# chenc10/distributed_TensorFlow_models

Measured on AMD Instinct MI355X. Metric: images/sec (whole node) ResNet-50 224×224 bf16 at 1/2/4/8 MI355X, higher is better.
Workload: dtype bf16; 1 GPU; model=resnet_v1_50, global_batch=256, per_gpu_batch=256, image_size=224, parallelism=dp1, device=cuda, grad_allreduce_dtype=fp32, deterministic=True, optimizer=momentum-sgd+wd

## Files before the change

csrc/kernels/conv_igemm.hip:

```cpp
#include "common.h"
#include <cstdio>

namespace dtm {


struct ConvNTArgs {
  const bf16_t* x;
  const bf16_t* w;
  bf16_t* y;
  float* stats;
  const float* bias;
  const float* in_scale;
  const float* in_shift;
  uint32_t x_bytes, w_bytes;
  int N, Hin, Win, C, K, R, S, P, Q;
  int stride, pad_h, pad_w;
  int Hv, Wv;
  int M;
  int Kg;
  int relu;
  FastDiv fd_PQ, fd_Q;
  const bf16_t* add_src;
  int add_stride;
  int add_H, add_W;
// ... 1139 lines not shown
          *(uint2*)(smem + mloc * OROW + kloc * 2) = make_uint2(pack2bf(v[0], v[1]), pack2bf(v[2], v[3]));
        }
    }
  conv_nt_epi_tail<PT, CT, false, false, false, 512, true, false, SPL>(a, smem, p0, c0, by, nullptr, nullptr);
}

template <int CT>
__device__ __forceinline__ void worker_row(float* red, const float* lo, const float* hi, float* row, int c0, int K) {
  constexpr int CPR = CT / 8, RPT = 256 / CPR;
  const int tid = threadIdx.x;
  __syncthreads();
#pragma unroll
  for (int e = 0; e < 8; ++e) { red[tid * 16 + e] = lo[e]; red[tid * 16 + 8 + e] = hi[e]; }
  __syncthreads();
  for (int h = RPT / 2; h >= 1; h >>= 1) {
    if (tid < h * CPR) {
#pragma unroll
      for (int e = 0; e < 16; ++e) red[tid * 16 + e] += red[(tid + h * CPR) * 16 + e];
    }
    __syncthreads();
  }
  const int kc = c0 + tid * 8;
  if (tid < CPR && kc < K) {
#pragma unroll
    for (int e = 0; e < 8; ++e) { row[kc + e] = red[tid * 16 + e]; row[K + kc + e] = red[tid * 16 + 8 + e]; }
  }
}

__device__ __forceinline__ void glds16(const void* gptr, const void* lds) {
  const uint32_t l = __builtin_amdgcn_readfirstlane((uint32_t)(uintptr_t)(const __attribute__((address_space(3))) void*)lds);
  asm volatile("s_mov_b32 m0, %1\n\ts_nop 0\n\tglobal_load_lds_dwordx4 %0, off" ::"v"(gptr), "s"(l) : "memory", "m0");
}

template <int PT, int CT, int NKT, bool PRO, bool STEM = false, int NBUF = 2, bool SIDE = true>
__global__ __launch_bounds__(256) void conv1x1_stream_kernel(ConvNTArgs a, int ntiles) {
  constexpr int WP = PT / 2, WC = CT / 2;
  constexpr int TP = WP / 16, TC = WC / 16;
  constexpr int AI = PT / 32, WI = CT / 32;
  constexpr int ABUF = NKT * PT * 128;
  constexpr int WBUF = NKT * CT * 128;
  constexpr int OROW = CT * 2 + 16;
  constexpr int STG = PT * OROW > 16384 ? PT * OROW : 16384;
  constexpr int NIT = PT * (CT / 8) / 256;
  constexpr int MAXC = 512;
  constexpr int OFF_A = WBUF, OFF_S = WBUF + NBUF * ABUF, OFF_P = OFF_S + STG;
  constexpr int NDMA = NKT * AI;
  static_assert(NBUF == 2 || NBUF == 3, "ring depth");
  static_assert(2 * NIT + NDMA <= 63, "vmcnt range");
  __shared__ __attribute__((aligned(16))) char smem[OFF_P + (PRO ? MAXC * 8 : 0)];
  typedef __attribute__((address_space(1))) const void gvoid;
  typedef __attribute__((address_space(3))) void lvoid;
  static_assert(NIT >= 1 && NIT <= 15, "vmcnt lower bound");

  const int tid = threadIdx.x, lane = tid & 63, wave = tid >> 6;
  const int nb = gridDim.x * gridDim.y;
  const int bid = xcd_remap(blockIdx.y * gridDim.x + blockIdx.x, nb);
  const int bx = bid % gridDim.x, by0 = bid / gridDim.x;
  const int c0 = bx * CT;
  const int lr = lane >> 3;
  const int ch = (lane & 7) ^ lr;
  const char* xg = (const char*)a.x;
  const char* wg = (const char*)a.w;
  const char* zg = (const char*)a.zero;
  float* s_scale = (float*)(smem + OFF_P);
  float* s_shift = s_scale + MAXC;
  if constexpr (PRO) {
    for (int c = tid; c < a.C; c += 256) { s_scale[c] = a.in_scale[c]; s_shift[c] = a.in_shift[c]; }
  }
#pragma unroll
  for (int kt = 0; kt < NKT; ++kt) {
#pragma unroll
    for (int j = 0; j < WI; ++j) {
      const int row = c0 + 8 * (wave + 4 * j) + lr;
      const int k = kt * 64 + ch * 8;
      const bool v = (row < a.K) & (k < a.Kg);
      const char* src = wg + (size_t)(uint32_t)((row * a.Kg + k) * 2);
      __builtin_amdgcn_global_load_lds((gvoid*)(v ? src : zg), (lvoid*)(smem + kt * CT * 128 + (wave + 4 * j) * 1024),
                                       16, 0, 0);
    }
  }
  const char* srcs[NKT * AI];
  auto issue = [&](int t, int buf) {
    char* base = smem + OFF_A + buf * ABUF;
    uint32_t pix[AI];
    if constexpr (STEM) {
#pragma unroll
      for (int j = 0; j < AI; ++j) {
        const int m = t * PT + 8 * (wave + 4 * j) + lr;
        const uint32_t mm = m < a.M ? (uint32_t)m : 0u;
        const uint32_t n = fdiv(mm, a.fd_PQ), rem = mm - n * (a.P * a.Q);
        const uint32_t p = fdiv(rem, a.fd_Q), q = rem - p * a.Q;
        pix[j] = ((n * a.Hin + p * a.stride) * a.Win + q * a.stride) * 8u;
      }
    }
#pragma unroll
    for (int kt = 0; kt < NKT; ++kt) {
      const int k = kt * 64 + ch * 8;
#pragma unroll
      for (int j = 0; j < AI; ++j) {
        const int m = t * PT + 8 * (wave + 4 * j) + lr;
        const bool v = (m < a.M) & (k < a.Kg);
        const char* src = STEM ? xg + (size_t)(pix[j] + (uint32_t)((k >> 5) * a.Win * 8 + (k & 31) * 2))
                               : xg + (size_t)(uint32_t)(m * a.pix_bytes + k * 2);
        srcs[kt * AI + j] = v ? src : zg;
        glds16(srcs[kt * AI + j], base + kt * PT * 128 + (wave + 4 * j) * 1024);
      }
    }
  };
  auto transform = [&](int t, int buf) {
    char* base = smem + OFF_A + buf * ABUF;
#pragma unroll
    for (int kt = 0; kt < NKT; ++kt) {
      const int k = kt * 64 + ch * 8;
      if (k < a.Kg) {
        const float4 s0 = *(const float4*)(s_scale + k), s1 = *(const float4*)(s_scale + k + 4);
        const float4 h0 = *(const float4*)(s_shift + k), h1 = *(const float4*)(s_shift + k + 4);
        const float sc[8] = {s0.x, s0.y, s0.z, s0.w, s1.x, s1.y, s1.z, s1.w};
        const float sh[8] = {h0.x, h0.y, h0.z, h0.w, h1.x, h1.y, h1.z, h1.w};
#pragma unroll
        for (int j = 0; j < AI; ++j) {
          const int m = t * PT + 8 * (wave + 4 * j) + lr;
          if (m < a.M) {
            uint4* pp = (uint4*)(base + kt * PT * 128 + (wave + 4 * j) * 1024 + lane * 16);
            const uint4 q = *pp;
            uint32_t u[4] = {q.x, q.y, q.z, q.w};
#pragma unroll
            for (int e = 0; e < 4; ++e) {
              const float lo = fmaxf(fmaf(lo_bf(u[e]), sc[2 * e], sh[2 * e]), 0.f);
              const float hi = fmaxf(fmaf(hi_bf(u[e]), sc[2 * e + 1], sh[2 * e + 1]), 0.f);
              u[e] = pack2bf(lo, hi);
            }
            *pp = make_uint4(u[0], u[1], u[2], u[3]);
          }
        }
      }
    }
  };

  const int wp = wave % 2, wc = wave / 2;
  const int fr = lane & 15, fk = lane >> 4;
  float ssum[8], ssq[8], aacc[24];
#pragma unroll
  for (int e = 0; e < 8; ++e) { ssum[e] = 0.f; ssq[e] = 0.f; }
#pragma unroll
  for (int e = 0; e < 24; ++e) aacc[e] = 0.f;
  int t = by0;
  const int gy = gridDim.y;
  if (t < ntiles) issue(t, 0);
  if (NBUF == 3 && t + gy < ntiles) issue(t + gy, 1);
  asm volatile("s_waitcnt vmcnt(0)" ::: "memory");
  __syncthreads();
  int buf = 0;
  for (int it = 0; t < ntiles; ++it, t += gy) {
    if constexpr (NBUF == 2) {
      if (it > 0) asm volatile("s_waitcnt vmcnt(%0)" ::"n"(NIT) : "memory");
    } else if (it >= 2) {
      if (t + gy < ntiles) asm volatile("s_waitcnt vmcnt(%0)" ::"n"(2 * NIT + NDMA) : "memory");
      else asm volatile("s_waitcnt vmcnt(%0)" ::"n"(2 * NIT) : "memory");
    }
    if constexpr (PRO) transform(t, buf);
    asm volatile("s_waitcnt lgkmcnt(0)" ::: "memory");
    __builtin_amdgcn_s_barrier();
    if constexpr (NBUF == 2) {
      if (t + gy < ntiles) issue(t + gy, buf ^ 1);
    } else {
      if (t + 2 * gy < ntiles) issue(t + 2 * gy, buf == 0 ? 2 : buf - 1);
    }
    f32x4 acc[TC][TP];
#pragma unroll
    for (int i = 0; i < TC; ++i)
#pragma unroll
      for (int j = 0; j < TP; ++j) acc[i][j] = (f32x4){0.f, 0.f, 0.f, 0.f};
    const char* abase = smem + OFF_A + buf * ABUF;
#pragma unroll
    for (int kt = 0; kt < NKT; ++kt) {
#pragma unroll
      for (int ks = 0; ks < 2; ++ks) {
        short8 bf[TP], af[TC];
        const int chn = ks * 4 + fk;
#pragma unroll
        for (int j = 0; j < TP; ++j) {
          const int row = wp * WP + j * 16 + fr;
          bf[j] = *(const short8*)(abase + kt * PT * 128 + row * 128 + ((chn ^ (row & 7)) << 4));
        }
#pragma unroll
        for (int i = 0; i < TC; ++i) {
          const int row = wc * WC + i * 16 + fr;
          af[i] = *(const short8*)(smem + kt * CT * 128 + row * 128 + ((chn ^ (row & 7)) << 4));
        }
#pragma unroll
        for (int i = 0; i < TC; ++i)
#pragma unroll
          for (int j = 0; j < TP; ++j)
            acc[i][j] = __builtin_amdgcn_mfma_f32_16x16x32_bf16(af[i], bf[j], acc[i][j], 0, 0, 0);
      }
    }
    conv_nt_epilogue<PT, CT, WP, WC, 1, true, true, true, true, 256, SIDE>(a, acc, smem + OFF_S, t * PT, c0, t, ssum,
                                                                           ssq, nullptr, nullptr, aacc);
#pragma unroll
    for (int i = 0; i < NKT * AI; ++i) asm volatile("" ::"v"(srcs[i]));
    buf = buf + 1 == NBUF ? 0 : buf + 1;
  }
  asm volatile("s_waitcnt vmcnt(0)" ::: "memory");
  if (a.stats) worker_row<CT>((float*)(smem + OFF_S), ssum, ssq, a.stats + (size_t)by0 * (2 * a.K), c0, a.K);
  if (SIDE && a.act_x && a.act_sums) {
    const int rw = a.act_r ? 4 : 2;
    float* row = a.act_sums + (size_t)by0 * (rw * a.K);
    worker_row<CT>((float*)(smem + OFF_S), aacc, aacc + 8, row, c0, a.K);
    if (a.act_r) worker_row<CT>((float*)(smem + OFF_S), aacc + 16, aacc + 8, row + 2 * a.K, c0, a.K);
  }
}

template <int CIN>
__device__ __forceinline__ int dsw(int p, int c) {
  return CIN == 64 ? (c ^ ((p >> 1) & 7)) : (c ^ ((p >> 2) & 3));
}

template <int CIN, int CT, bool SIDE>
__global__ __launch_bounds__(256) void conv3x3_direct_kernel(ConvNTArgs a, int ntiles) {
  constexpr int TH = 8, TW = 16, PT = TH * TW, HH = TH + 2, HW = TW + 2;
  constexpr int CPP = CIN / 8;
  constexpr int HCH = HH * HW * CPP;
  constexpr int NDMA = (HCH + 255) / 256;
  constexpr int OROW = CT * 2 + 16;
  constexpr int HDMA = NDMA * 256 * 16;
  constexpr int HBUF = HDMA > PT * OROW ? HDMA : PT * OROW;
  static_assert(3 * HBUF >= 256 * 16 * 4, "worker_row's reduction table fits in the ring");
  constexpr int WBUF = 9 * CT * CIN * 2;
  constexpr int NIT = PT * (CT / 8) / 256;
  constexpr int TC = CT / 16, TP = 2;
  constexpr int SD = SIDE ? 2 * NIT : 0;
  constexpr int SBUF = SIDE ? 2 * NIT * 4096 + 2 * CT * 4 : 0;
  static_assert(2 * NIT + SD + NDMA <= 63, "vmcnt range");
  __shared__ __attribute__((aligned(16))) char smem[WBUF + 3 * HBUF + SBUF];
  char* sside = smem + WBUF + 3 * HBUF;
  float* s_ss = (float*)(sside + 2 * NIT * 4096);

  const int tid = threadIdx.x, lane = tid & 63, wave = tid >> 6;
  const int nb = gridDim.x * gridDim.y;
  const int bid = xcd_remap(blockIdx.y * gridDim.x + blockIdx.x, nb);
  const int bx = bid % gridDim.x, by0 = bid / gridDim.x;
  const int c0 = bx * CT;
// ... 1016 lines not shown
  }
  return (const bf16_t*)z;
}
const void* dtm_zero_chunk() { return zero_chunk(); }

template <int PT, int CT, int NWP, int NS, int UD, bool SPL = false, int NTH = 512>
static void launch_w8(const ConvNTArgs& a, hipStream_t st) {
  dim3 grid((a.K + CT - 1) / CT, (a.M + PT - 1) / PT, a.ngrp > 1 ? a.ngrp : 1);
  hipLaunchKernelGGL((conv_nt_w8_kernel<PT, CT, NWP, NS, UD, SPL, NTH>), grid, dim3(NTH), 0, st, a);
}

template <int UD, bool SPL = false>
static void launch_pp(const ConvNTArgs& a, hipStream_t st) {
  dim3 grid((a.K + 255) / 256, (a.M + 255) / 256, a.ngrp > 1 ? a.ngrp : 1);
  hipLaunchKernelGGL((conv_nt_pp_kernel<UD, SPL>), grid, dim3(512), 0, st, a);
}

template <int PT, int CT, int NS, int UD, int NWP = 2, bool SPL = false>
static void launch_pipe(const ConvNTArgs& a, hipStream_t st) {
  dim3 grid((a.K + CT - 1) / CT, (a.M + PT - 1) / PT, a.ngrp > 1 ? a.ngrp : 1);
  if (SPL) hipLaunchKernelGGL((conv_nt_pipe_kernel<PT, CT, NS, UD, false, NWP, true>), grid, dim3(256), 0, st, a);
  else if (a.in_scale) hipLaunchKernelGGL((conv_nt_pipe_kernel<PT, CT, NS, UD, true, NWP>), grid, dim3(256), 0, st, a);
  else hipLaunchKernelGGL((conv_nt_pipe_kernel<PT, CT, NS, UD, false, NWP>), grid, dim3(256), 0, st, a);
}

static int device_cus() { return dtm_compute_cus(); }

static bf16_t* dump_chunk() {
  static void* z = nullptr;
  if (!z && hipMalloc(&z, 4096) != hipSuccess) return nullptr;
  return (bf16_t*)z;
}

template <int PT, int CT, int NKT, bool PRO, bool STEM = false, int NBUF = 2, bool SIDE = true>
static int stream_workers_k(const ConvNTArgs& a) {
  static int occ = 0;
  if (!occ) {
    if (hipOccupancyMaxActiveBlocksPerMultiprocessor(&occ, conv1x1_stream_kernel<PT, CT, NKT, PRO, STEM, NBUF, SIDE>,
                                                     256, 0) !=
            hipSuccess || occ <= 0)
      occ = 1;
  }
  const int ctiles = (a.K + CT - 1) / CT;
  const int ntiles = (a.M + PT - 1) / PT;
  int workers = (occ * device_cus() + ctiles - 1) / ctiles;
  if (workers > ntiles) workers = ntiles;
  if (workers < 1) workers = 1;
  return workers;
}

template <int PT, int CT, int NKT, bool PRO, bool STEM = false, int NBUF = 2, bool SIDE = true>
static void launch_stream_k(const ConvNTArgs& a, hipStream_t st) {
  const int ctiles = (a.K + CT - 1) / CT;
  const int ntiles = (a.M + PT - 1) / PT;
  hipLaunchKernelGGL((conv1x1_stream_kernel<PT, CT, NKT, PRO, STEM, NBUF, SIDE>),
                     dim3(ctiles, stream_workers_k<PT, CT, NKT, PRO, STEM, NBUF, SIDE>(a)), dim3(256), 0, st, a, ntiles);
}

static bool stem_stream_ok(const ConvNTArgs& a) {
  return a.pix_bytes == 8 && a.C == 32 && a.S == 1 && a.pad_h == 0 && a.pad_w == 0 && a.Kg == a.R * 32 &&
         a.Kg <= 256 && a.K % 64 == 0 && !a.in_scale && !a.bias && !a.relu && a.ostr == 1;
}

template <int CT, int NKT>
static void launch_stream(const ConvNTArgs& a, hipStream_t st) {
  const bool side = a.add_src || a.act_x;
  if (a.in_scale) {
    if (side) launch_stream_k<64, CT, NKT, true, false, 2, true>(a, st);
    else launch_stream_k<64, CT, NKT, true, false, 2, false>(a, st);
  } else if (side) launch_stream_k<64, CT, NKT, false, false, 2, true>(a, st);
  else launch_stream_k<64, CT, NKT, false, false, 2, false>(a, st);
}
template <int CT, int NKT>
static int stream_workers(const ConvNTArgs& a) {
  const bool side = a.add_src || a.act_x;
  if (a.in_scale) return side ? stream_workers_k<64, CT, NKT, true, false, 2, true>(a)
                              : stream_workers_k<64, CT, NKT, true, false, 2, false>(a);
  if (side) return stream_workers_k<64, CT, NKT, false, false, 2, true>(a);
  return stream_workers_k<64, CT, NKT, false, false, 2, false>(a);
}

static int g_stem_stream = 1;
DTM_API void dtm_conv_set_stem_stream(int on) { g_stem_stream = on; }
static int stream_rows(const ConvNTArgs& a, int id) {
  if (id == 33) return g_stem_stream == 2 ? stream_workers_k<64, 64, 4, false, true, 2, false>(a)
                                          : stream_workers_k<64, 64, 4, false, true, 3, false>(a);
  const bool k1 = a.Kg <= 64;
  if (id == 30) {
    return k1 ? stream_workers<128, 1>(a) : stream_workers<128, 2>(a);
  }
  return k1 ? stream_workers<64, 1>(a) : stream_workers<64, 2>(a);
}

static bool stream_ok(const ConvNTArgs& a) {
  return !a.bias && !a.relu && a.R == 1 && a.S == 1 && a.stride == 1 && a.pad_h == 0 && a.pad_w == 0 && a.Hv == a.Hin && a.Wv == a.Win &&
         a.P == a.Hin && a.Q == a.Win && a.Kg % 64 == 0 && a.Kg <= 128 && a.K % 8 == 0 &&
         (!a.in_scale || a.C <= 512) && a.dump != nullptr && a.ostr == 1;
}

template <int PT, int CT, int WP, int WC, int UD, int NBUF = 2, bool SPL = false, int LBW = 0, int EG = 4, int BO = 0>
static void launch_nt(const ConvNTArgs& a, hipStream_t st) {
  dim3 grid((a.K + CT - 1) / CT, (a.M + PT - 1) / PT, a.ngrp > 1 ? a.ngrp : 1);
  hipLaunchKernelGGL((conv_nt_kernel<PT, CT, WP, WC, UD, NBUF, SPL, LBW, EG, BO>), grid, dim3(256), 0, st, a);
}
static int g_act_occ = getenv("DTM_ACT_OCC") ? atoi(getenv("DTM_ACT_OCC")) : 2;
DTM_API void dtm_conv_set_act_occ(int v) { g_act_occ = v; }
static int g_nt_occ = getenv("DTM_NT_OCC") ? atoi(getenv("DTM_NT_OCC")) : 2;
DTM_API void dtm_conv_set_nt_occ(int v) { g_nt_occ = v; }
template <int PT, int CT, int UD>
static void launch_nt_act(const ConvNTArgs& a, hipStream_t st) {
  const bool side = (a.K & 7) == 0 && (a.add_src != nullptr || a.act_x != nullptr);
  const int v = side ? g_act_occ : (a.stats ? 0 : g_nt_occ);
  if (v == 1) launch_nt<PT, CT, 32, 64, UD, 1, false, 0, 2>(a, st);
  else if (v == 2) launch_nt<PT, CT, 32, 64, UD, 1, false, 4, 4>(a, st);
  else if (v == 3) launch_nt<PT, CT, 32, 64, UD, 1, false, 4, 2>(a, st);
  else launch_nt<PT, CT, 32, 64, UD, 1>(a, st);
}

static int g_direct3 = 1;
DTM_API void dtm_conv_set_direct3(int on) { g_direct3 = on; }
static bool direct_ok(const ConvNTArgs& a) {
  return a.R == 3 && a.S == 3 && a.stride == 1 && a.Hv == a.Hin && a.Wv == a.Win && (a.C == 32 || a.C == 64) &&
         a.K % 32 == 0 && !a.in_scale && !a.bias && !a.relu && a.pix_bytes == a.C * 2 && a.ostr == 1 &&
         a.pad_h <= 2 && a.pad_w <= 2 && !a.act_mask && !a.act_r && (!a.add_src || a.add_stride == 1);
}
static void direct_setup(ConvNTArgs& a) {
  a.sp_tw = (a.Q + 15) / 16;
  a.sp_th = (a.P + 7) / 8;
  a.fd_sp_img = make_fastdiv(a.sp_th * a.sp_tw);
// ... 15 lines not shown
}
template <int CIN, int CT, bool SIDE>
static void launch_direct_k(const ConvNTArgs& a, hipStream_t st) {
  hipLaunchKernelGGL((conv3x3_direct_kernel<CIN, CT, SIDE>), dim3(a.K / CT, direct_workers_k<CIN, CT, SIDE>(a)),
                     dim3(256), 0, st, a, a.M / 128);
}
static int g_direct_ct32 = getenv("DTM_DIRECT_CT32") ? atoi(getenv("DTM_DIRECT_CT32")) : 1;
DTM_API void dtm_conv_set_direct_ct32(int on) { g_direct_ct32 = on; }
#define DTM_DIRECT_SEL(FN, ...)                                                                     \
  ((a.add_src || a.act_x)                                                                          \
       ? (a.C == 64 ? FN<64, 32, true>(__VA_ARGS__) : FN<32, 32, true>(__VA_ARGS__))                 \
       : (a.C == 64 ? ((a.K % 64 == 0 && !g_direct_ct32) ? FN<64, 64, false>(__VA_ARGS__)           \
                                                        : FN<64, 32, false>(__VA_ARGS__))           \
                    : ((a.K % 64 == 0 && !g_direct_ct32) ? FN<32, 64, false>(__VA_ARGS__)           \
                                                        : FN<32, 32, false>(__VA_ARGS__))))
static int direct_workers(const ConvNTArgs& a) { return DTM_DIRECT_SEL(direct_workers_k, a); }
static void launch_direct(const ConvNTArgs& a, hipStream_t st) { DTM_DIRECT_SEL(launch_direct_k, a, st); }

struct TileCfg {
  int id, PT, NWP;
};
static int g_tile_env = -2;
static int g_last_nt_tile = -1, g_last_wgrad_tile = -1;
DTM_API void dtm_conv_last_tiles(int* nt, int* wgrad) {
  if (nt) *nt = g_last_nt_tile;
  if (wgrad) *wgrad = g_last_wgrad_tile;
}
static int device_cus();
static int g_policy2 = 1;
DTM_API void dtm_conv_set_policy2(int on) { g_policy2 = on; }
static int g_tile_w8 = 1;
static int g_stream_act = 0;
DTM_API void dtm_conv_set_stream_act(int on) { g_stream_act = on; }
static int g_kwide = 1;
DTM_API void dtm_conv_set_kwide(int on) { g_kwide = on; }
DTM_API void dtm_conv_set_w8(int on) { g_tile_w8 = on; }
static int g_tile_pp = getenv("DTM_PP") ? atoi(getenv("DTM_PP")) : 0;
DTM_API void dtm_conv_set_pp(int on) { g_tile_pp = on; }
static int g_k64_tile = 3;
DTM_API void dtm_conv_set_k64_tile(int id) { g_k64_tile = id; }
static int g_k32_tile = 1;
DTM_API void dtm_conv_set_k32(int on) { g_k32_tile = on; }
static int g_act_tile = -1;
DTM_API void dtm_conv_set_act_tile(int id) { g_act_tile = id; }
static TileCfg pick_tile_impl(const ConvNTArgs& a, bool stats);
static TileCfg pick_tile(const ConvNTArgs& a, bool stats = false) {
  static int log = -1;
  if (log < 0) {
    const char* e = getenv("DTM_TILE_LOG");
    log = e ? atoi(e) : 0;
  }
  const TileCfg t = pick_tile_impl(a, stats);
  if (log)
    fprintf(stderr, "dtm_tile M=%d K=%d C=%d RxS=%dx%d Kg=%d st=%d ostr=%d pro=%d stats=%d add=%d act=%d mask=%d r=%d -> %d\n",
            a.M, a.K, a.C, a.R, a.S, a.Kg, a.stride, a.ostr, a.in_scale != nullptr, (int)stats, a.add_src != nullptr,
            a.act_x != nullptr, a.act_mask != nullptr, a.act_r != nullptr, t.id);
  return t;
}
static TileCfg pick_tile_impl(const ConvNTArgs& a, bool stats) {
  if (g_tile_env == -2) {
    const char* e = getenv("DTM_CONV_TILE");
    g_tile_env = e ? atoi(e) : -1;
  }
  int id = g_tile_env;
  if (id == -1 && g_stem_stream && stem_stream_ok(a)) return {33, 64, 2};
  if (((id == -1 && a.K == 32) || id == 60) && g_direct3 && direct_ok(a)) return {60, 128, 4};
  if (id == -1 && a.K == 64 && a.C == 32 && !a.in_scale && g_direct3 && direct_ok(a)) return {60, 128, 4};
  if (id == -4) id = -1;
  else if (id == -1 && a.Kg == 64 && stream_ok(a) && (g_stream_act || !a.act_x) &&
           (!g_policy2 || a.K % 128 == 0 || a.K <= 64))
    id = a.K >= 128 ? 30 : 31;
  if (id == -1 && a.act_x && g_act_tile >= 0) id = g_act_tile;
  if (id == -1 && !a.in_scale && a.K >= 256 && g_tile_w8 && (!g_policy2 || a.K % 256 == 0)) {
    const long tiles = (long)((a.M + 255) / 256) * ((a.K + 255) / 256);
    if (tiles >= 150 && !(tiles > 600 && a.Kg <= 256 && !stats)) id = 40;
  }
  if (id == -1 && g_policy2 && !a.in_scale && a.K % 8 == 0 && a.R * a.S > 1) {
    if (a.K <= 32 && g_k32_tile) id = 32;
    else if (a.K <= 64) id = 26;
    else if (a.K <= 128) id = 21;
  }
  if (id == -1 && g_kwide && a.K > 64 && a.K % 128 != 0 && (a.K % 128) <= 64 && a.K % 8 == 0)
    id = a.in_scale ? 3 : ((g_policy2 && a.M >= 16384 && (a.M <= 65536 || a.M >= 262144)) ? 24 : 26);
  if (id == -1 && !a.in_scale && a.Kg >= 1024) {
    id = 21;
    if (g_policy2 && (long)((a.M + 127) / 128) * ((a.K + 127) / 128) <= device_cus()) id = 26;
  }
  if (id == -1 && !a.in_scale && a.K <= 64 && a.R * a.S > 1 && a.K % 64 == 0) id = 26;
  if (id < 0) id = a.K <= 64 ? g_k64_tile : ((a.M <= 16384 && a.Kg >= 2048) ? 0 : 4);
  if ((id == 21 || id == 24 || id == 26 || id == 32) && a.in_scale && a.C > 512) id = 0;
  if (id == 21 || id == 26) return {id, 128, 2};
  if (id == 24) return {id, 256, 2};
  if (id == 32) return {id, 256, 4};
  if ((id == 40 || id == 41) && a.in_scale) id = 0;
  if (id == 40 && g_tile_pp && g_tile_env != 40) id = 41;
  if (id == 41 && a.K % 8) id = 40;
  if (id == 40 || id == 41) return {id, 256, 2};
  if (id == 30 || id == 31) {
    if (stream_ok(a)) return {id, 64, 2};
    id = a.K <= 64 ? 3 : 4;
  }
  if (id == 3) return {id, 128, 4};
  if (id == 4) return {id, 64, 2};
  return {0, 128, 2};
}

static void dispatch_split(const ConvNTArgs& a, const TileCfg& t, hipStream_t st) {
  const int id = t.id;
  g_last_nt_tile = (id == 3 || id == 4 || id == 21 || id == 24 || id == 26 || id == 32 || id == 40 || id == 41) ? id : 0;
  if (t.id == 3) launch_nt<128, 64, 32, 64, 1, 1, true>(a, st);
  else if (t.id == 4) launch_nt<64, 128, 32, 64, 1, 1, true>(a, st);
  else if (t.id == 21) launch_pipe<128, 128, 2, 1, 2, true>(a, st);
  else if (t.id == 24) launch_pipe<256, 64, 2, 1, 2, true>(a, st);
  else if (t.id == 26) launch_pipe<128, 64, 2, 1, 2, true>(a, st);
  else if (t.id == 32) launch_pipe<256, 32, 2, 1, 4, true>(a, st);
  else if (t.id == 40) launch_w8<256, 256, 2, 2, 1, true>(a, st);
  else if (t.id == 41) launch_pp<1, true>(a, st);
  else launch_nt<128, 128, 64, 64, 1, 2, true>(a, st);
}

template <int UD>
static void dispatch_ud(const ConvNTArgs& a, const TileCfg& t, hipStream_t st) {
  if (UD == 1 && a.nsplit > 0) dispatch_split(a, t, st);
  else if (t.id == 3) launch_nt_act<128, 64, UD>(a, st);
  else if (t.id == 4) launch_nt_act<64, 128, UD>(a, st);
  else if (t.id == 30 && UD == 1) {
    if (a.Kg <= 64) launch_stream<128, 1>(a, st);
    else launch_stream<128, 2>(a, st);
  } else if (t.id == 60 && UD == 1) {
    launch_direct(a, st);
  } else if (t.id == 33 && UD == 1) {
    if (g_stem_stream == 2) launch_stream_k<64, 64, 4, false, true, 2, false>(a, st);
    else launch_stream_k<64, 64, 4, false, true, 3, false>(a, st);
  } else if (t.id == 31 && UD == 1) {
    if (a.Kg <= 64) launch_stream<64, 1>(a, st);
    else launch_stream<64, 2>(a, st);
  } else if (t.id == 21) launch_pipe<128, 128, 2, UD>(a, st);
  else if (t.id == 24) launch_pipe<256, 64, 2, UD>(a, st);
  else if (t.id == 26) launch_pipe<128, 64, 2, UD>(a, st);
  else if (t.id == 32) launch_pipe<256, 32, 2, UD, 4>(a, st);
  else if (t.id == 40) launch_w8<256, 256, 2, 2, UD>(a, st);
  else if (t.id == 41) launch_pp<UD>(a, st);
  else launch_nt<128, 128, 64, 64, UD>(a, st);
}

DTM_API void dtm_conv_set_tile(int id) { g_tile_env = id; }

static void dispatch_nt(const ConvNTArgs& a, int ud, const TileCfg& t, hipStream_t st) {
  g_last_nt_tile = (ud != 1 && (t.id == 30 || t.id == 31 || t.id == 33 || t.id == 60)) ? 0 : t.id;
  if (ud == 1) dispatch_ud<1>(a, t, st);
  else dispatch_ud<2>(a, t, st);
}

DTM_API int dtm_get_deterministic();

static int g_split_tile = 1;
DTM_API void dtm_conv_set_split_tile(int on) { g_split_tile = on; }

static int g_blockout = -1, g_blockout_nt = 1;
DTM_API void dtm_conv_set_blockout(int mode, int nt) { g_blockout = mode; g_blockout_nt = nt; }
struct BlockOut {
  const void* res;
  const float* ss;
  const float* rss;
  void* y;
  void* mask;
};
constexpr int DTM_DECLINED = 1;
static void launch_blockout(const ConvNTArgs& a, int tile, hipStream_t st) {
  g_last_nt_tile = tile == 3 ? 3 : 4;
  if (tile == 3) {
    if (g_blockout_nt) launch_nt<128, 64, 32, 64, 1, 1, false, 3, 4, 2>(a, st);
    else launch_nt<128, 64, 32, 64, 1, 1, false, 3, 4, 1>(a, st);
  } else {
    if (g_blockout_nt) launch_nt<64, 128, 32, 64, 1, 1, false, 3, 4, 2>(a, st);
    else launch_nt<64, 128, 32, 64, 1, 1, false, 3, 4, 1>(a, st);
  }
}

static int conv_fwd_impl(const void* x, const void* w, void* y, bool stats, const float* bias, const float* in_scale,
                         const float* in_shift, int relu, const ConvDesc* d, hipStream_t stream, float** rows_ws,
                         int* nrows, const ConvNTArgs::Split* split = nullptr, int nsplit = 0,
// ... 2 lines not shown
  if (d->C % 8 || d->K % 4) return -1;
  ConvNTArgs a;
  a.x = (const bf16_t*)x; a.w = (const bf16_t*)w; a.y = (bf16_t*)y;
  a.ngrp = 0;
  a.nsplit = 0;
  a.stats = nullptr; a.bias = bias; a.in_scale = in_scale; a.in_shift = in_shift;
  a.add_src = nullptr; a.act_x = nullptr; a.act_ss = nullptr; a.act_sums = nullptr;
  a.act_mask = nullptr; a.act_r = nullptr;
  a.add_stride = 1; a.add_H = a.add_W = 0;
  a.act_unscaled = 0;
  a.zero = zero_chunk();
  a.dump = dump_chunk();
  a.pix_bytes = d->pix_bytes > 0 ? d->pix_bytes : d->C * 2;
  size_t xb = (size_t)d->N * d->H * d->W * a.pix_bytes, wb = (size_t)d->K * d->R * d->S * d->C * 2;
  if (xb >= (1ull << 31) || wb >= (1ull << 31)) return -2;
  a.x_bytes = (uint32_t)xb; a.w_bytes = (uint32_t)wb;
  a.N = d->N; a.Hin = d->H; a.Win = d->W; a.C = d->C; a.K = d->K; a.R = d->R; a.S = d->S;
  a.P = d->P; a.Q = d->Q; a.stride = d->stride; a.pad_h = d->pad_h; a.pad_w = d->pad_w;
  a.Hv = d->H; a.Wv = d->W;
  a.M = d->N * d->P * d->Q; a.Kg = d->R * d->S * d->C; a.relu = relu;
  a.fd_PQ = make_fastdiv(d->P * d->Q); a.fd_Q = make_fastdiv(d->Q);
  a.ostr = 1; a.oa = a.ob = 0; a.OH = a.P; a.OW = a.Q;
  a.sp_tw = a.sp_th = 0;
  if (nsplit > 0) {
    if (nsplit > 8 || d->K % 8) return -1;
    a.nsplit = nsplit;
    for (int i = 0; i < nsplit; ++i) {
      if (split[i].off % 8 || split[i].K % 8) return -1;
      a.split[i] = split[i];
    }
  }
  int rows = 0;
  TileCfg tc = pick_tile(a, stats);
  if (nsplit > 0 && (tc.id == 30 || tc.id == 31 || tc.id == 33 || tc.id == 60)) tc = {4, 64, 2};
  if (nsplit > 0 && g_split_tile && g_tile_env < 0 && tc.id != 40 && tc.id != 21) tc = {21, 128, 2};
  if (bo) {
    const int ct = tc.id == 3 ? 64 : 128;
    if (g_blockout == 0 || (tc.id != 3 && tc.id != 4) || (g_blockout == 2 && tc.id != 3) ||
        (g_blockout == 3 && tc.id != 4) || a.K > ct || a.R != 1 || a.S != 1 || a.stride != 1 ||
        a.pad_h || a.pad_w || a.P != a.Hin || a.Q != a.Win || a.C % 8 || a.C > 512 || a.pix_bytes != a.C * 2 ||
        bias || relu || in_scale || nsplit > 0 || !stats || !bo->res || !bo->ss || !bo->y)
      return DTM_DECLINED;
    a.bo_res = (const bf16_t*)bo->res; a.bo_ss = bo->ss; a.bo_rss = bo->rss;
    a.bo_y = (bf16_t*)bo->y; a.bo_mask = (uint8_t*)bo->mask;
  }
  if (tc.id == 60) direct_setup(a);
  if (stats) {
    rows = tc.id == 60 ? direct_workers(a)
           : (tc.id == 30 || tc.id == 31 || tc.id == 33) ? stream_rows(a, tc.id)
                                                          : ((a.M + tc.PT - 1) / tc.PT) * ((a.K & 7) == 0 ? 1 : tc.NWP);
    float* ws = dtm_ws_get_stream((size_t)rows * 2 * d->K, stream);
    if (!ws) return -4;
    a.stats = ws;
  }
  if (bo) launch_blockout(a, tc.id, stream);
  else dispatch_nt(a, 1, tc, stream);
  *rows_ws = a.stats;
  *nrows = rows;
  return 0;
}

DTM_API int dtm_conv_fwd(const void* x, const void* w, void* y, float* stats, const float* bias,
                         const float* in_scale, const float* in_shift, int relu,
                         const ConvDesc* d, void* stream) {
  float* ws = nullptr;
  int rows = 0;
  int rc = conv_fwd_impl(x, w, y, stats != nullptr, bias, in_scale, in_shift, relu, d, (hipStream_t)stream, &ws, &rows);
  if (rc) return rc;
  if (stats) dtm_reduce_rows(ws, rows, 2 * d->K, 2 * d->K, stats, (hipStream_t)stream);
  return 0;
}

DTM_API int dtm_conv_fwd_bn_multi(const void* x, const void* w, void* const* ys, const int* ks, int n,
                                  void* const* bn_ptrs, float count, float eps, float decay, int update, int bessel,
                                  const ConvDesc* d, void* stream) {
  if (n < 1 || n > 8) return -1;
  ConvNTArgs::Split sp[8];
  FinGroup fg;
  fg.n = n;
  int off = 0;
  for (int i = 0; i < n; ++i) {
    sp[i].y = (bf16_t*)ys[i];
// ... 102 lines not shown
  const int st = d->stride;
  const bool dec = d->dec && st > 1;
  if (!dec && st > 2) return -3;
  if (dec && (d->R < st || d->S < st)) return -8;
  ConvNTArgs la[16];
  TileCfg lt[16];
  int lrows[16], nl = 0, rows = 0;
  for (int ca = 0; ca < (dec ? st : 1); ++ca)
    for (int cb = 0; cb < (dec ? st : 1); ++cb) {
      ConvNTArgs b = a;
      if (dec) {
        int r0, Tr, offa, s0, Tu, offb;
        dec_dim(d->R, st, d->pad_h, ca, r0, Tr, offa);
        dec_dim(d->S, st, d->pad_w, cb, s0, Tu, offb);
        const int Hc = (d->H - ca + st - 1) / st, Wc = (d->W - cb + st - 1) / st;
        if (Hc <= 0 || Wc <= 0) continue;
        b.w = (const bf16_t*)wt + dec_block(d->R, d->S, d->C, d->K, st, d->pad_h, d->pad_w, ca, cb);
        b.R = Tr; b.S = Tu;
        b.P = Hc; b.Q = Wc;
        b.pad_h = Tr - 1 - offa; b.pad_w = Tu - 1 - offb;
        b.ostr = st; b.oa = ca; b.ob = cb;
      } else {
        b.R = d->R; b.S = d->S;
        b.P = d->H; b.Q = d->W;
        b.pad_h = d->R - 1 - d->pad_h; b.pad_w = d->S - 1 - d->pad_w;
        b.Hv = (d->P - 1) * st + 1; b.Wv = (d->Q - 1) * st + 1;
        b.ostr = 1; b.oa = b.ob = 0;
      }
      b.M = d->N * b.P * b.Q; b.Kg = b.R * b.S * d->K;
      b.fd_PQ = make_fastdiv(b.P * b.Q); b.fd_Q = make_fastdiv(b.Q);
      lt[nl] = pick_tile(b);
      if (lt[nl].id == 60) direct_setup(b);
      lrows[nl] = lt[nl].id == 60 ? direct_workers(b)
                  : (lt[nl].id == 30 || lt[nl].id == 31) ? stream_rows(b, lt[nl].id)
                                                         : (b.M + lt[nl].PT - 1) / lt[nl].PT;
      rows += lrows[nl];
      la[nl++] = b;
    }
  int gi = -1;
  if (dec && nl > 1 && nl <= 4 && g_dec_group) {
    gi = 0;
    for (int i = 1; i < nl; ++i) {
      if (la[i].M != la[0].M || la[i].P != la[0].P || la[i].Q != la[0].Q) gi = -2;
      if (gi >= 0 && la[i].Kg > la[gi].Kg) gi = i;
    }
    int id = gi >= 0 ? lt[gi].id : -1;
    if (gi >= 0 && g_dec_tile && (id == 21 || id == 26) && g_tile_env < 0 && g_act_tile < 0) {
      if (la[gi].K % 256 == 0 && g_tile_w8) lt[gi] = {g_tile_pp ? 41 : 40, 256, 2};
      else if (la[gi].K <= 128) lt[gi] = {26, 128, 2};
      id = lt[gi].id;
    }
    if (!(id == 0 || id == 3 || id == 4 || id == 21 || id == 24 || id == 26 || id == 32 || id == 40 || id == 41)) gi = -1;
    if (gi >= 0) {
      rows = 0;
      for (int i = 0; i < nl; ++i) {
        lt[i] = lt[gi];
        lrows[i] = (la[i].M + lt[gi].PT - 1) / lt[gi].PT;
        rows += lrows[i];
      }
    }
  }
  float* ws = nullptr;
  if (act_x) {
    ws = dtm_ws_get_stream((size_t)rows * rw * d->C, (hipStream_t)stream);
    if (!ws) return -4;
  }
  for (int i = 0, r = 0; i < nl; r += lrows[i], ++i)
// ... 257 lines not shown
```

distributed_tensorflow_models_amd/ops/_lib.py:

```python
import ctypes
import os

import torch

_HERE = os.path.dirname(os.path.dirname(os.path.abspath(__file__)))
LIB_PATH = os.environ.get("DTM_KERNELS_SO") or os.path.join(_HERE, "_native", "libdtm_kernels.so")

_lib = None


class ConvDesc(ctypes.Structure):
    _fields_ = [(n, ctypes.c_int) for n in
                ("N", "H", "W", "C", "K", "R", "S", "P", "Q", "stride", "pad_h", "pad_w", "pix_bytes", "dec")]


class PoolArgs(ctypes.Structure):
    _fields_ = [(n, ctypes.c_int) for n in
                ("N", "H", "W", "C", "P", "Q", "KH", "KW", "SH", "SW", "PH", "PW")]


_P = ctypes.c_void_p
_I = ctypes.c_int
_L = ctypes.c_long
_F = ctypes.c_float
# ... 110 lines not shown
    "dtm_bn_finalize_bwd": (None, [_P, _P, _P, _P, _P, _P, _I, _F, _P]),
    "dtm_lrn": (_I, [_P, _P, _P, _L, _I, _I, _F, _F, _F, _I, _P]),
    "dtm_ws_reserve": (_I, [_L]),
    "dtm_ws_last_error": (_I, []),
    "dtm_ws_retired": (_L, []),
    "dtm_ws_reserve_stream": (_I, [_L, _P]),
    "dtm_ws_capacity": (_L, [_P]),
    "dtm_depthwise_fwd": (_I, [_P, _P, _P, _P, _P]),
    "dtm_depthwise_dgrad": (_I, [_P, _P, _P, _P, _P]),
    "dtm_depthwise_wgrad": (_I, [_P, _P, _P, _P, _P]),
    "dtm_set_reduce_policy": (None, [_I, _I, _I]),
    "dtm_bn_apply_ld": (_I, [_P, _P, _P, _P, _L, _I, _I, _I, _P]),
    "dtm_bn_apply_bwd_ld": (_I, [_P, _P, _P, _P, _P, _P, _L, _I, _I, _I, _P]),
    "dtm_set_sc_policy": (None, [_I, _I]),
    "dtm_set_ntld_policy": (None, [_I]),
    "dtm_set_deterministic": (None, [_I]),
    "dtm_get_deterministic": (_I, []),
    "dtm_conv_set_k64_tile": (None, [_I]),
    "dtm_conv_set_w8": (None, [_I]),
    "dtm_conv_set_kwide": (None, [_I]),
    "dtm_set_reduce_few": (None, [_I]),
    "dtm_set_reserved_cus": (None, [_I]),
    "dtm_stats_combine_multi": (_I, [_P, _P, _I, _F, _P, _L, _I, _P]),
    "dtm_conv_fwd_bn_multi": (_I, [_P, _P, _P, _P, _I, _P, _F, _F, _F, _I, _I, ctypes.POINTER(ConvDesc), _P]),
    "dtm_conv_fwd_bn_blockout": (_I, [_P] * 13 + [_F, _F, _F, _I, _I, ctypes.POINTER(ConvDesc), _P]),
    "dtm_conv_set_blockout": (None, [_I, _I]),
    "dtm_conv_set_dec_lpt": (None, [_I]),
    "dtm_conv_set_dec_tile": (None, [_I]),
    "dtm_conv_set_split_tile": (None, [_I]),
    "dtm_get_reserved_cus": (_I, []),
    "dtm_compute_cus_api": (_I, []),
    "dtm_cu_hog": (_I, [_I, _F, _P]),
    "dtm_conv_set_stream_act": (None, [_I]),
    "dtm_conv_set_act_tile": (None, [_I]),
    "dtm_stem_pack": (_I, [_P, _I, _P, _I, _I, _I, _I, _I, _I, _I, _P]),
    "dtm_dropout": (_I, [_P, _P, _L, _I, _F, ctypes.c_ulonglong, _P, _P]),
    "dtm_in_top_k": (_I, [_P, _P, _P, _I, _I, _I, _I, _P]),
    "dtm_stats_tensor_bytes": (_I, []),
    "dtm_stats_chunk_bytes": (_I, []),
    "dtm_stats_partial_bytes": (_I, []),
    "dtm_stats_result_bytes": (_I, []),
    "dtm_stats_chunk_size": (_I, []),
    "dtm_stats_num_buckets": (_I, []),
    "dtm_stats_limits": (None, [_P]),
    "dtm_tensor_stats": (_I, [_P, _P, _I, _I, _P, _P, _P, _P]),
    "dtm_metrics_header_words": (_I, []),
    "dtm_metrics_max_classes": (_I, []),
    "dtm_metrics_max_confusion_classes": (_I, []),
    "dtm_metrics_max_batch": (_I, []),
    "dtm_eval_metrics": (_I, [_P, _I, _P, _I, _I, _I, _I, _I, _P, _P, _P, _P]),
    "dtm_fq_rec_words": (_I, []),
    "dtm_fq_partial_stride": (_I, []),
    "dtm_fq_threads": (_I, []),
    "dtm_fq_grid": (_I, [_L, _I]),
    "dtm_fq_range": (_I, [_P, _I, _L, _P, _P]),
    "dtm_fq_finalize": (_I, [_P, _I, _P, _P, _P, _P, _I, _F, _F, _I, _I, _L, _I, _P]),
    "dtm_fq_apply": (_I, [_P, _P, _I, _L, _P, _P]),
    "dtm_fq_apply_bwd": (_I, [_P, _P, _P, _I, _L, _P, _P]),
    "dtm_fq_advance": (_I, [_P, _P]),
}


def gpu_present():
    try:
        return torch.cuda.is_available()
    except Exception:
# ... 138 lines not shown
```

Measured before the change: 15730 images/sec.

## Add 8-wave persistent stream 1x1 conv kernel for Kg 128/256 with grouped stats rows

Generalizes the streaming 1x1 conv kernel to 512 threads (8 waves) and adds two new tile ids (34, 35) that use it for 1x1 convs with Kg 128 or 256 and K divisible by 256. Each worker walks groups of four 64-row tiles and writes one deterministic BN-stats row per 256 output rows, so stats match the existing 256-row partition. The weight tile stays resident in LDS while activation tiles stream through a double buffer. This aims to cut the weight reloads and tile launch overhead of the generic tiled path. In exchange it adds per-group reductions and barriers, and it uses more LDS per block.

```diff
diff --git a/csrc/kernels/conv_igemm.hip b/csrc/kernels/conv_igemm.hip
--- a/csrc/kernels/conv_igemm.hip
+++ b/csrc/kernels/conv_igemm.hip
@@ -1195,18 +1195,25 @@
   asm volatile("s_mov_b32 m0, %1\n\ts_nop 0\n\tglobal_load_lds_dwordx4 %0, off" ::"v"(gptr), "s"(l) : "memory", "m0");
 }
 
-template <int PT, int CT, int NKT, bool PRO, bool STEM = false, int NBUF = 2, bool SIDE = true>
-__global__ __launch_bounds__(256) void conv1x1_stream_kernel(ConvNTArgs a, int ntiles) {
-  constexpr int WP = PT / 2, WC = CT / 2;
+template <int PT, int CT, int NKT, bool PRO, bool STEM = false, int NBUF = 2, bool SIDE = true, int NT = 256>
+__global__ __launch_bounds__(NT) void conv1x1_stream_kernel(ConvNTArgs a, int ntiles) {
+  constexpr int NW = NT / 64;
+  static_assert(NT == 256 || (NT == 512 && !SIDE && !STEM), "4 waves, or the 8-wave forward form");
+  constexpr int WP = PT / 2, WC = CT / (NW / 2);
   constexpr int TP = WP / 16, TC = WC / 16;
-  constexpr int AI = PT / 32, WI = CT / 32;
+  constexpr int AI = PT / (8 * NW), WI = CT / (8 * NW);
+  static_assert(AI >= 1 && WI >= 1 && PT % (8 * NW) == 0 && CT % (8 * NW) == 0, "whole DMA pieces per wave");
   constexpr int ABUF = NKT * PT * 128;
   constexpr int WBUF = NKT * CT * 128;
   constexpr int OROW = CT * 2 + 16;
   constexpr int STG = PT * OROW > 16384 ? PT * OROW : 16384;
-  constexpr int NIT = PT * (CT / 8) / 256;
+  constexpr int NIT = PT * (CT / 8) / NT;
   constexpr int MAXC = 512;
   constexpr int OFF_A = WBUF, OFF_S = WBUF + NBUF * ABUF, OFF_P = OFF_S + STG;
+  constexpr bool TR = NT == 512;
+  constexpr int NSTAT = (CT / 8) * 16;
+  static_assert(!TR || (NBUF == 2 && PT == 64 && NSTAT <= NT && STG >= NSTAT * 64), "group rows: table in the staging area");
+  static_assert(OFF_P + (PRO ? MAXC * 8 : 0) <= 160 * 1024, "LDS budget");
   constexpr int NDMA = NKT * AI;
   static_assert(NBUF == 2 || NBUF == 3, "ring depth");
   static_assert(2 * NIT + NDMA <= 63, "vmcnt range");
@@ -1228,17 +1235,17 @@
   float* s_scale = (float*)(smem + OFF_P);
   float* s_shift = s_scale + MAXC;
   if constexpr (PRO) {
-    for (int c = tid; c < a.C; c += 256) { s_scale[c] = a.in_scale[c]; s_shift[c] = a.in_shift[c]; }
+    for (int c = tid; c < a.C; c += NT) { s_scale[c] = a.in_scale[c]; s_shift[c] = a.in_shift[c]; }
   }
 #pragma unroll
   for (int kt = 0; kt < NKT; ++kt) {
 #pragma unroll
     for (int j = 0; j < WI; ++j) {
-      const int row = c0 + 8 * (wave + 4 * j) + lr;
+      const int row = c0 + 8 * (wave + NW * j) + lr;
       const int k = kt * 64 + ch * 8;
       const bool v = (row < a.K) & (k < a.Kg);
       const char* src = wg + (size_t)(uint32_t)((row * a.Kg + k) * 2);
-      __builtin_amdgcn_global_load_lds((gvoid*)(v ? src : zg), (lvoid*)(smem + kt * CT * 128 + (wave + 4 * j) * 1024),
+      __builtin_amdgcn_global_load_lds((gvoid*)(v ? src : zg), (lvoid*)(smem + kt * CT * 128 + (wave + NW * j) * 1024),
                                        16, 0, 0);
     }
   }
@@ -1249,7 +1256,7 @@
     if constexpr (STEM) {
 #pragma unroll
       for (int j = 0; j < AI; ++j) {
-        const int m = t * PT + 8 * (wave + 4 * j) + lr;
+        const int m = t * PT + 8 * (wave + NW * j) + lr;
         const uint32_t mm = m < a.M ? (uint32_t)m : 0u;
         const uint32_t n = fdiv(mm, a.fd_PQ), rem = mm - n * (a.P * a.Q);
         const uint32_t p = fdiv(rem, a.fd_Q), q = rem - p * a.Q;
@@ -1261,12 +1268,12 @@
       const int k = kt * 64 + ch * 8;
 #pragma unroll
       for (int j = 0; j < AI; ++j) {
-        const int m = t * PT + 8 * (wave + 4 * j) + lr;
+        const int m = t * PT + 8 * (wave + NW * j) + lr;
         const bool v = (m < a.M) & (k < a.Kg);
         const char* src = STEM ? xg + (size_t)(pix[j] + (uint32_t)((k >> 5) * a.Win * 8 + (k & 31) * 2))
                                : xg + (size_t)(uint32_t)(m * a.pix_bytes + k * 2);
         srcs[kt * AI + j] = v ? src : zg;
-        glds16(srcs[kt * AI + j], base + kt * PT * 128 + (wave + 4 * j) * 1024);
+        glds16(srcs[kt * AI + j], base + kt * PT * 128 + (wave + NW * j) * 1024);
       }
     }
   };
@@ -1282,9 +1289,9 @@
         const float sh[8] = {h0.x, h0.y, h0.z, h0.w, h1.x, h1.y, h1.z, h1.w};
 #pragma unroll
         for (int j = 0; j < AI; ++j) {
-          const int m = t * PT + 8 * (wave + 4 * j) + lr;
+          const int m = t * PT + 8 * (wave + NW * j) + lr;
           if (m < a.M) {
-            uint4* pp = (uint4*)(base + kt * PT * 128 + (wave + 4 * j) * 1024 + lane * 16);
+            uint4* pp = (uint4*)(base + kt * PT * 128 + (wave + NW * j) * 1024 + lane * 16);
             const uint4 q = *pp;
             uint32_t u[4] = {q.x, q.y, q.z, q.w};
 #pragma unroll
@@ -1307,14 +1314,15 @@
   for (int e = 0; e < 8; ++e) { ssum[e] = 0.f; ssq[e] = 0.f; }
 #pragma unroll
   for (int e = 0; e < 24; ++e) aacc[e] = 0.f;
-  int t = by0;
   const int gy = gridDim.y;
+  int t = TR ? 4 * by0 : by0;
+  auto nxt = [&](int u) { return TR ? ((u & 3) == 3 ? u + 4 * gy - 3 : u + 1) : u + gy; };
   if (t < ntiles) issue(t, 0);
   if (NBUF == 3 && t + gy < ntiles) issue(t + gy, 1);
   asm volatile("s_waitcnt vmcnt(0)" ::: "memory");
   __syncthreads();
   int buf = 0;
-  for (int it = 0; t < ntiles; ++it, t += gy) {
+  for (int it = 0; t < ntiles; ++it, t = nxt(t)) {
     if constexpr (NBUF == 2) {
       if (it > 0) asm volatile("s_waitcnt vmcnt(%0)" ::"n"(NIT) : "memory");
     } else if (it >= 2) {
@@ -1325,7 +1333,7 @@
     asm volatile("s_waitcnt lgkmcnt(0)" ::: "memory");
     __builtin_amdgcn_s_barrier();
     if constexpr (NBUF == 2) {
-      if (t + gy < ntiles) issue(t + gy, buf ^ 1);
+      if (nxt(t) < ntiles) issue(nxt(t), buf ^ 1);
     } else {
       if (t + 2 * gy < ntiles) issue(t + 2 * gy, buf == 0 ? 2 : buf - 1);
     }
@@ -1358,19 +1366,68 @@
             acc[i][j] = __builtin_amdgcn_mfma_f32_16x16x32_bf16(af[i], bf[j], acc[i][j], 0, 0, 0);
       }
     }
-    conv_nt_epilogue<PT, CT, WP, WC, 1, true, true, true, true, 256, SIDE>(a, acc, smem + OFF_S, t * PT, c0, t, ssum,
-                                                                           ssq, nullptr, nullptr, aacc);
+    float dsum[8], dsq[8];
+#pragma unroll
+    for (int e = 0; e < 8; ++e) { dsum[e] = 0.f; dsq[e] = 0.f; }
+    constexpr bool OWN = TR && CT != 256;
+    conv_nt_epilogue<PT, CT, WP, WC, 1, true, true, true, true, NT, SIDE>(a, acc, smem + OFF_S, t * PT, c0, t,
+                                                                          OWN ? dsum : ssum, OWN ? dsq : ssq, nullptr,
+                                                                          nullptr, aacc);
+    if constexpr (TR) {
+      if (a.stats) {
+        constexpr int CPR = CT / 8;
+        if constexpr (OWN) {
+          if (tid < NSTAT) {
+            const int c = tid % CPR, g = tid / CPR;
+            const int kc = c0 + c * 8;
+#pragma unroll
+            for (int j = 0; j < 4; ++j) {
+              const int row = g + 16 * j;
+              if (t * PT + row < a.M && kc < a.K) {
+                const uint4 v = *(const uint4*)(smem + OFF_S + row * OROW + c * 16);
+                const float q[8] = {lo_bf(v.x), hi_bf(v.x), lo_bf(v.y), hi_bf(v.y),
+                                    lo_bf(v.z), hi_bf(v.z), lo_bf(v.w), hi_bf(v.w)};
+#pragma unroll
+                for (int e = 0; e < 8; ++e) { ssum[e] += q[e]; ssq[e] = fmaf(q[e], q[e], ssq[e]); }
+              }
+            }
+          }
+        }
+        if ((t & 3) == 3) {
+          epi_barrier<true>();
+          float* red = (float*)(smem + OFF_S);
+          if (tid < NSTAT) {
+#pragma unroll
+            for (int e = 0; e < 8; ++e) { red[tid * 16 + e] = ssum[e]; red[tid * 16 + 8 + e] = ssq[e]; }
+          }
+          epi_barrier<true>();
+          float* prow = a.stats + (size_t)(t >> 2) * (2 * a.K);
+          for (int o = tid; o < CPR * 16; o += NT) {
+            const int c = o >> 4, e = o & 15;
+            float r = 0.f;
+#pragma unroll 4
+            for (int k = 0; k < 16; ++k) r += red[((c + k * CPR) << 4) + e];
+            const int kk = c0 + c * 8 + (e & 7);
+            if (kk < a.K) prow[(e < 8 ? 0 : a.K) + kk] = r;
+          }
+#pragma unroll
+          for (int e = 0; e < 8; ++e) { ssum[e] = 0.f; ssq[e] = 0.f; }
+        }
+      }
+    }
 #pragma unroll
     for (int i = 0; i < NKT * AI; ++i) asm volatile("" ::"v"(srcs[i]));
     buf = buf + 1 == NBUF ? 0 : buf + 1;
   }
   asm volatile("s_waitcnt vmcnt(0)" ::: "memory");
-  if (a.stats) worker_row<CT>((float*)(smem + OFF_S), ssum, ssq, a.stats + (size_t)by0 * (2 * a.K), c0, a.K);
-  if (SIDE && a.act_x && a.act_sums) {
-    const int rw = a.act_r ? 4 : 2;
-    float* row = a.act_sums + (size_t)by0 * (rw * a.K);
-    worker_row<CT>((float*)(smem + OFF_S), aacc, aacc + 8, row, c0, a.K);
-    if (a.act_r) worker_row<CT>((float*)(smem + OFF_S), aacc + 16, aacc + 8, row + 2 * a.K, c0, a.K);
+  if constexpr (!TR) {
+    if (a.stats) worker_row<CT>((float*)(smem + OFF_S), ssum, ssq, a.stats + (size_t)by0 * (2 * a.K), c0, a.K);
+    if (SIDE && a.act_x && a.act_sums) {
+      const int rw = a.act_r ? 4 : 2;
+      float* row = a.act_sums + (size_t)by0 * (rw * a.K);
+      worker_row<CT>((float*)(smem + OFF_S), aacc, aacc + 8, row, c0, a.K);
+      if (a.act_r) worker_row<CT>((float*)(smem + OFF_S), aacc + 16, aacc + 8, row + 2 * a.K, c0, a.K);
+    }
   }
 }
 
@@ -2453,29 +2510,32 @@
   return (bf16_t*)z;
 }
 
-template <int PT, int CT, int NKT, bool PRO, bool STEM = false, int NBUF = 2, bool SIDE = true>
+static int g_stream_workers_cap = 0;
+DTM_API void dtm_conv_set_stream_workers_cap(int n) { g_stream_workers_cap = n; }
+template <int PT, int CT, int NKT, bool PRO, bool STEM = false, int NBUF = 2, bool SIDE = true, int NT = 256>
 static int stream_workers_k(const ConvNTArgs& a) {
   static int occ = 0;
   if (!occ) {
-    if (hipOccupancyMaxActiveBlocksPerMultiprocessor(&occ, conv1x1_stream_kernel<PT, CT, NKT, PRO, STEM, NBUF, SIDE>,
-                                                     256, 0) !=
+    if (hipOccupancyMaxActiveBlocksPerMultiprocessor(&occ, conv1x1_stream_kernel<PT, CT, NKT, PRO, STEM, NBUF, SIDE, NT>,
+                                                     NT, 0) !=
             hipSuccess || occ <= 0)
       occ = 1;
   }
   const int ctiles = (a.K + CT - 1) / CT;
-  const int ntiles = (a.M + PT - 1) / PT;
+  const int ntiles = NT == 512 ? (a.M + 255) / 256 : (a.M + PT - 1) / PT;
   int workers = (occ * device_cus() + ctiles - 1) / ctiles;
+  if (g_stream_workers_cap > 0 && workers > g_stream_workers_cap) workers = g_stream_workers_cap;
   if (workers > ntiles) workers = ntiles;
   if (workers < 1) workers = 1;
   return workers;
 }
 
-template <int PT, int CT, int NKT, bool PRO, bool STEM = false, int NBUF = 2, bool SIDE = true>
+template <int PT, int CT, int NKT, bool PRO, bool STEM = false, int NBUF = 2, bool SIDE = true, int NT = 256>
 static void launch_stream_k(const ConvNTArgs& a, hipStream_t st) {
   const int ctiles = (a.K + CT - 1) / CT;
-  const int ntiles = (a.M + PT - 1) / PT;
-  hipLaunchKernelGGL((conv1x1_stream_kernel<PT, CT, NKT, PRO, STEM, NBUF, SIDE>),
-                     dim3(ctiles, stream_workers_k<PT, CT, NKT, PRO, STEM, NBUF, SIDE>(a)), dim3(256), 0, st, a, ntiles);
+  const int ntiles = NT == 512 ? 4 * ((a.M + 255) / 256) : (a.M + PT - 1) / PT;
+  hipLaunchKernelGGL((conv1x1_stream_kernel<PT, CT, NKT, PRO, STEM, NBUF, SIDE, NT>),
+                     dim3(ctiles, stream_workers_k<PT, CT, NKT, PRO, STEM, NBUF, SIDE, NT>(a)), dim3(NT), 0, st, a, ntiles);
 }
 
 static bool stem_stream_ok(const ConvNTArgs& a) {
@@ -2501,9 +2561,16 @@
   return stream_workers_k<64, CT, NKT, false, false, 2, false>(a);
 }
 
+template <int CT, int NKT>
+static void launch_stream8(const ConvNTArgs& a, hipStream_t st) {
+  if (a.in_scale) launch_stream_k<64, CT, NKT, true, false, 2, false, 512>(a, st);
+  else launch_stream_k<64, CT, NKT, false, false, 2, false, 512>(a, st);
+}
+
 static int g_stem_stream = 1;
 DTM_API void dtm_conv_set_stem_stream(int on) { g_stem_stream = on; }
 static int stream_rows(const ConvNTArgs& a, int id) {
+  if (id == 34 || id == 35) return (a.M + 255) / 256;
   if (id == 33) return g_stem_stream == 2 ? stream_workers_k<64, 64, 4, false, true, 2, false>(a)
                                           : stream_workers_k<64, 64, 4, false, true, 3, false>(a);
   const bool k1 = a.Kg <= 64;
@@ -2513,9 +2580,11 @@
   return k1 ? stream_workers<64, 1>(a) : stream_workers<64, 2>(a);
 }
 
-static bool stream_ok(const ConvNTArgs& a) {
+static bool stream_ok(const ConvNTArgs& a, int id = 30) {
+  const int kmax = id == 35 ? 256 : 128;
+  if ((id == 34 || id == 35) && (a.add_src || a.act_x)) return false;
   return !a.bias && !a.relu && a.R == 1 && a.S == 1 && a.stride == 1 && a.pad_h == 0 && a.pad_w == 0 && a.Hv == a.Hin && a.Wv == a.Win &&
-         a.P == a.Hin && a.Q == a.Win && a.Kg % 64 == 0 && a.Kg <= 128 && a.K % 8 == 0 &&
+         a.P == a.Hin && a.Q == a.Win && a.Kg % 64 == 0 && a.Kg <= kmax && a.K % 8 == 0 &&
          (!a.in_scale || a.C <= 512) && a.dump != nullptr && a.ostr == 1;
 }
 
@@ -2597,6 +2666,8 @@
 static int g_tile_w8 = 1;
 static int g_stream_act = 0;
 DTM_API void dtm_conv_set_stream_act(int on) { g_stream_act = on; }
+static int g_stream8 = 3;
+DTM_API void dtm_conv_set_stream8(int classes) { g_stream8 = classes; }
 static int g_kwide = 1;
 DTM_API void dtm_conv_set_kwide(int on) { g_kwide = on; }
 DTM_API void dtm_conv_set_w8(int on) { g_tile_w8 = on; }
@@ -2635,6 +2706,10 @@
   else if (id == -1 && a.Kg == 64 && stream_ok(a) && (g_stream_act || !a.act_x) &&
            (!g_policy2 || a.K % 128 == 0 || a.K <= 64))
     id = a.K >= 128 ? 30 : 31;
+  else if (id == -1 && stats && !a.in_scale && g_tile_w8 && a.K % 256 == 0 &&
+           (long)((a.M + 255) / 256) * (a.K / 256) >= 150 &&
+           (((g_stream8 & 1) && a.Kg == 128 && stream_ok(a, 34)) || ((g_stream8 & 2) && a.Kg == 256 && stream_ok(a, 35))))
+    id = a.Kg == 128 ? 34 : 35;
   if (id == -1 && a.act_x && g_act_tile >= 0) id = g_act_tile;
   if (id == -1 && !a.in_scale && a.K >= 256 && g_tile_w8 && (!g_policy2 || a.K % 256 == 0)) {
     const long tiles = (long)((a.M + 255) / 256) * ((a.K + 255) / 256);
@@ -2661,8 +2736,8 @@
   if (id == 40 && g_tile_pp && g_tile_env != 40) id = 41;
   if (id == 41 && a.K % 8) id = 40;
   if (id == 40 || id == 41) return {id, 256, 2};
-  if (id == 30 || id == 31) {
-    if (stream_ok(a)) return {id, 64, 2};
+  if (id == 30 || id == 31 || id == 34 || id == 35) {
+    if (stream_ok(a, id)) return {id, 64, 2};
     id = a.K <= 64 ? 3 : 4;
   }
   if (id == 3) return {id, 128, 4};
@@ -2692,6 +2767,10 @@
   else if (t.id == 30 && UD == 1) {
     if (a.Kg <= 64) launch_stream<128, 1>(a, st);
     else launch_stream<128, 2>(a, st);
+  } else if (t.id == 34 && UD == 1) {
+    launch_stream8<256, 2>(a, st);
+  } else if (t.id == 35 && UD == 1) {
+    launch_stream8<128, 4>(a, st);
   } else if (t.id == 60 && UD == 1) {
     launch_direct(a, st);
   } else if (t.id == 33 && UD == 1) {
@@ -2712,7 +2791,7 @@
 DTM_API void dtm_conv_set_tile(int id) { g_tile_env = id; }
 
 static void dispatch_nt(const ConvNTArgs& a, int ud, const TileCfg& t, hipStream_t st) {
-  g_last_nt_tile = (ud != 1 && (t.id == 30 || t.id == 31 || t.id == 33 || t.id == 60)) ? 0 : t.id;
+  g_last_nt_tile = (ud != 1 && (t.id == 30 || t.id == 31 || t.id == 33 || t.id == 34 || t.id == 35 || t.id == 60)) ? 0 : t.id;
   if (ud == 1) dispatch_ud<1>(a, t, st);
   else dispatch_ud<2>(a, t, st);
 }
@@ -2781,7 +2860,7 @@
   }
   int rows = 0;
   TileCfg tc = pick_tile(a, stats);
-  if (nsplit > 0 && (tc.id == 30 || tc.id == 31 || tc.id == 33 || tc.id == 60)) tc = {4, 64, 2};
+  if (nsplit > 0 && (tc.id == 30 || tc.id == 31 || tc.id == 33 || tc.id == 34 || tc.id == 35 || tc.id == 60)) tc = {4, 64, 2};
   if (nsplit > 0 && g_split_tile && g_tile_env < 0 && tc.id != 40 && tc.id != 21) tc = {21, 128, 2};
   if (bo) {
     const int ct = tc.id == 3 ? 64 : 128;
@@ -2796,7 +2875,7 @@
   if (tc.id == 60) direct_setup(a);
   if (stats) {
     rows = tc.id == 60 ? direct_workers(a)
-           : (tc.id == 30 || tc.id == 31 || tc.id == 33) ? stream_rows(a, tc.id)
+           : (tc.id == 30 || tc.id == 31 || (tc.id >= 33 && tc.id <= 35)) ? stream_rows(a, tc.id)
                                                           : ((a.M + tc.PT - 1) / tc.PT) * ((a.K & 7) == 0 ? 1 : tc.NWP);
     float* ws = dtm_ws_get_stream((size_t)rows * 2 * d->K, stream);
     if (!ws) return -4;
@@ -2965,7 +3044,7 @@
       lt[nl] = pick_tile(b);
       if (lt[nl].id == 60) direct_setup(b);
       lrows[nl] = lt[nl].id == 60 ? direct_workers(b)
-                  : (lt[nl].id == 30 || lt[nl].id == 31) ? stream_rows(b, lt[nl].id)
+                  : (lt[nl].id == 30 || lt[nl].id == 31 || lt[nl].id == 34 || lt[nl].id == 35) ? stream_rows(b, lt[nl].id)
                                                          : (b.M + lt[nl].PT - 1) / lt[nl].PT;
       rows += lrows[nl];
       la[nl++] = b;
diff --git a/distributed_tensorflow_models_amd/ops/_lib.py b/distributed_tensorflow_models_amd/ops/_lib.py
--- a/distributed_tensorflow_models_amd/ops/_lib.py
+++ b/distributed_tensorflow_models_amd/ops/_lib.py
@@ -166,6 +166,8 @@
     "dtm_compute_cus_api": (_I, []),
     "dtm_cu_hog": (_I, [_I, _F, _P]),
     "dtm_conv_set_stream_act": (None, [_I]),
+    "dtm_conv_set_stream8": (None, [_I]),
+    "dtm_conv_set_stream_workers_cap": (None, [_I]),
     "dtm_conv_set_act_tile": (None, [_I]),
     "dtm_stem_pack": (_I, [_P, _I, _P, _I, _I, _I, _I, _I, _I, _I, _P]),
     "dtm_dropout": (_I, [_P, _P, _L, _I, _F, ctypes.c_ulonglong, _P, _P]),
```

Measured after the change: 15930 images/sec (median of 6 runs). 1.01x the previous value.
